# benattal/neural-radiance-caching

Measured on AMD Instinct MI355X. Metric: rays/sec (1024-ray batch, 64+64 proposal + 32 shaded samples/ray), hotdog cache forward, higher is better.
Workload: dtype f32

## Files before the change

### neural-radiance-caching_amd/csrc/rc_dev_mlp.h

```cpp
#pragma once
#include "rc_internal.h"

namespace rcdev {

typedef float f32x16 __attribute__((ext_vector_type(16)));

constexpr int kWaves = 4;

__device__ __forceinline__ f32x16 zero16() {
  f32x16 z;
#pragma unroll
  for (int i = 0; i < 16; ++i) z[i] = 0.0f;
  return z;
}

typedef uint32_t u32x4 __attribute__((ext_vector_type(4)));
typedef __bf16 bf16x8 __attribute__((ext_vector_type(8)));

__device__ __forceinline__ uint32_t pack_top16(float a1, float a0) {
  return __builtin_amdgcn_perm(__float_as_uint(a1), __float_as_uint(a0), 0x07060302u);
}
__device__ __forceinline__ float top16(float a) { return __uint_as_float(__float_as_uint(a) & 0xffff0000u); }
__device__ __forceinline__ void split8(const float (&v)[8], u32x4 (&b)[3]) {
  u32x4 &hi = b[0], &mid = b[1], &lo = b[2];
#pragma unroll
  for (int p = 0; p < 4; ++p) {
    const float a0 = v[2 * p], a1 = v[2 * p + 1];
    hi[p] = pack_top16(a1, a0);
    const float r0 = a0 - top16(a0), r1 = a1 - top16(a1);
    mid[p] = pack_top16(r1, r0);
    const float l0 = r0 - top16(r0), l1 = r1 - top16(r1);
    lo[p] = pack_top16(l1, l0);
  }
}
__device__ __forceinline__ f32x16 mfma_bf16(const u32x4& a, const u32x4& b, const f32x16& c) {
  return __builtin_amdgcn_mfma_f32_32x32x16_bf16(__builtin_bit_cast(bf16x8, a), __builtin_bit_cast(bf16x8, b), c, 0, 0, 0);
}
#ifndef RC_RULE1
#define RC_RULE1 1
#endif
#ifndef RC_RULE2
#define RC_RULE2 1
#endif
#ifndef RC_RULE3
#define RC_RULE3 1
#endif
typedef float f32x4 __attribute__((ext_vector_type(4)));
__device__ __forceinline__ void split_fence() { if constexpr (RC_RULE1 != 0) __builtin_amdgcn_sched_barrier(0); }
__device__ __forceinline__ void split_keep(const u32x4& x) { if constexpr (RC_RULE2 != 0) asm volatile("" ::"v"(x)); }
__device__ __forceinline__ void split_keep3(const u32x4 (&x)[3]) { if constexpr (RC_RULE2 != 0) asm volatile("" ::"v"(x[0]), "v"(x[1]), "v"(x[2])); }
template <class WS>
__device__ __forceinline__ void split_flush(const WS& w, const u32x4& any) {
  if constexpr (RC_RULE3 == 0) return;
  __builtin_amdgcn_sched_barrier(0);
  w.sink = __builtin_amdgcn_mfma_f32_16x16x32_bf16(__builtin_bit_cast(bf16x8, any), __builtin_bit_cast(bf16x8, any), w.sink, 0, 0, 0);
  w.sink = __builtin_amdgcn_mfma_f32_16x16x32_bf16(__builtin_bit_cast(bf16x8, any), __builtin_bit_cast(bf16x8, any), w.sink, 0, 0, 0);
  __builtin_amdgcn_sched_barrier(0);
  asm volatile("s_nop 1" : "+v"(w.sink));
  __builtin_amdgcn_sched_barrier(0);
}
__device__ __forceinline__ void split_exclusive_simd() {
  if constexpr (kRcSplit) asm volatile("" ::: "v255", "a255");
}
__device__ __forceinline__ void mfma_split6(const u32x4 (&a)[3], const u32x4 (&b)[3], f32x16& acc) {
  split_fence();
  acc = mfma_bf16(a[2], b[0], acc);
  acc = mfma_bf16(a[0], b[2], acc);
  acc = mfma_bf16(a[1], b[1], acc);
  acc = mfma_bf16(a[1], b[0], acc);
  acc = mfma_bf16(a[0], b[1], acc);
  acc = mfma_bf16(a[0], b[0], acc);
  split_fence();
}

__device__ __forceinline__ void mfma_split3(const u32x4 (&a)[3], const u32x4& b0, f32x16& acc) {
  split_fence();
  acc = mfma_bf16(a[2], b0, acc);
  acc = mfma_bf16(a[1], b0, acc);
  acc = mfma_bf16(a[0], b0, acc);
  split_fence();
}

constexpr int kChunk = 64;
constexpr int kRingFloats = 2 * kChunk * 64;

typedef __attribute__((address_space(3))) void* lds_void_ptr;

struct WStream {
  const float* g;
  float* ring;
  int lane, wave;
  mutable f32x4 sink = {0.0f, 0.0f, 0.0f, 0.0f};
  __device__ WStream() = default;
  __device__ WStream(const float* g_, float* ring_, int lane_, int wave_) : g(g_), ring(ring_), lane(lane_), wave(wave_) {}
};

template <int NF, int W = kWaves, int CH = kChunk>
__device__ __forceinline__ void ws_issue(const WStream& w, int c) {
  static_assert(CH % (4 * W) == 0, "whole 1-KiB pieces per wave");
#pragma unroll
  for (int k = 0; k < CH / 4 / W; ++k) {
    const int i = w.wave + W * k;
    const int frag0 = c * CH + 4 * i;
    if (frag0 < NF) {
      const float* src = w.g + (size_t)frag0 * 64 + w.lane * 4;
      float* dst = w.ring + ((c & 1) * CH + 4 * i) * 64;
      __builtin_amdgcn_global_load_lds((const void*)src, (lds_void_ptr)dst, 16, 0, 0);
    }
  }
}

template <int NF, int W = kWaves, int CH = kChunk>
__device__ __forceinline__ void ws_begin(const WStream& w) {
  ws_issue<NF, W, CH>(w, 0);
  asm volatile("s_waitcnt vmcnt(0)" ::: "memory");
  __syncthreads();
  if (CH < NF) ws_issue<NF, W, CH>(w, 1);
}

template <int NF, int W = kWaves, int CH = kChunk>
__device__ __forceinline__ void ws_advance(const WStream& w, int c) {
  asm volatile("s_waitcnt vmcnt(0)" ::: "memory");
  __syncthreads();
  if ((c + 1) * CH < NF) ws_issue<NF, W, CH>(w, c + 1);
}

template <int NF, int W = kWaves, int CH = kChunk>
__device__ __forceinline__ float ws_read(const WStream& w, int f) {
  if (f > 0 && f % CH == 0) ws_advance<NF, W, CH>(w, f / CH);
  return w.ring[(f % (2 * CH)) * 64 + w.lane];
}

__device__ __forceinline__ u32x4 lds_piece(const float* p) { return *reinterpret_cast<const u32x4*>(p); }
template <int NF, int W = kWaves, int CH = kChunk>
__device__ __forceinline__ u32x4 ws_read4(const WStream& w, int f) {
  static_assert(CH % 4 == 0, "pieces never straddle a chunk");
  if (f > 0 && f % CH == 0) ws_advance<NF, W, CH>(w, f / CH);
  return lds_piece(w.ring + (f % (2 * CH)) * 64 + w.lane * 4);
}

struct WDirect {
  const float* g;
  int lane;
  mutable f32x4 sink = {0.0f, 0.0f, 0.0f, 0.0f};
};
template <int NF, int W = kWaves, int CH = kChunk>
__device__ __forceinline__ float ws_read(const WDirect& w, int f) { return w.g[(size_t)f * 64 + w.lane]; }
template <int NF, int W = kWaves, int CH = kChunk>
__device__ __forceinline__ u32x4 ws_read4(const WDirect& w, int f) { return *reinterpret_cast<const u32x4*>(w.g + (size_t)f * 64 + w.lane * 4); }

template <int NT, int KS, int FBASE, int NF, int SG, int W, int CH, class WS>
__device__ __forceinline__ void mlp_layer_f32(const WS& w, const float* act, f32x16 (&acc)[NT]) {
  constexpr int NG = (KS + SG - 1) / SG;
  float a[3][SG][NT], b[3][SG];
  auto load = [&](int g, int buf) {
#pragma unroll
    for (int d = 0; d < SG; ++d) {
      const int s = g * SG + d;
      if (s < KS) {
        b[buf][d] = act[s * 64];
#pragma unroll
        for (int t = 0; t < NT; ++t) {
          const int f = FBASE + s * NT + t;
          a[buf][d][t] = ws_read<NF, W, CH>(w, f);
        }
      }
    }
  };
  auto comp = [&](int g, int buf) {
#pragma unroll
    for (int d = 0; d < SG; ++d) {
      if (g * SG + d < KS) {
#pragma unroll
        for (int t = 0; t < NT; ++t)
          acc[t] = __builtin_amdgcn_mfma_f32_32x32x2f32(a[buf][d][t], b[buf][d], acc[t], 0, 0, 0);
      }
    }
  };
  load(0, 0);
  if (NG > 1) load(1, 1);
#pragma unroll
  for (int g = 0; g < NG; ++g) {
    if (g + 2 < NG) load(g + 2, (g + 2) % 3);
    __builtin_amdgcn_sched_barrier(0);
    comp(g, g % 3);
    __builtin_amdgcn_sched_barrier(0);
  }
}


template <int NBP>
__device__ __forceinline__ void split_blocks(const float* act, u32x4 (&pre)[NBP][3]) {
  float v[NBP][8];
#pragma unroll
  for (int q = 0; q < NBP; ++q)
#pragma unroll
    for (int j = 0; j < 8; ++j) v[q][j] = act[(8 * q + j) * 64];
#pragma unroll
  for (int q = 0; q < NBP; ++q) split8(v[q], pre[q]);
}
template <int NT, int KS, int FBASE, int NF, int W, int CH, int NBP, bool BIAS1, class WS>
__device__ __forceinline__ void mlp_layer_split(const WS& w, const float* act, f32x16 (&acc)[NT], const u32x4 (*pre)[3]) {
  static_assert(FBASE % 4 == 0, "split layers start on a 1-KiB piece");
  constexpr int NB = (KS + 7) / 8, NC = NB * NT;
  static_assert(NBP <= NB, "no more ready blocks than blocks");
  static_assert(!BIAS1 || KS % 8 == 1, "a bias block holds the bias step alone");
  float bv[8];
  u32x4 a[3][3], b[2][3];
  u32x4 b1;
  b1[0] = (BIAS1 && w.lane < 32) ? 0x00003f80u : 0u; b1[1] = 0u; b1[2] = 0u; b1[3] = 0u;
  auto from_act = [](int q) { return q < NB && q >= NBP && !(BIAS1 && q == NB - 1); };
  auto load_b = [&](int q) {
#pragma unroll
    for (int j = 0; j < 8; ++j) bv[j] = (8 * q + j < KS) ? act[(8 * q + j) * 64] : 0.0f;
  };
  auto load_a = [&](int cell) {
#pragma unroll
    for (int p = 0; p < 3; ++p) a[cell % 3][p] = ws_read4<NF, W, CH>(w, FBASE + (cell * 3 + p) * 4);
  };
  auto keep_b = [&](int q) {
    if (BIAS1 && q == NB - 1) split_keep(b1);
    else if (q < NBP) split_keep3(pre[q]);
    else split_keep3(b[q & 1]);
  };
  if (from_act(0)) load_b(0);
  load_a(0);
  if (NC > 1) load_a(1);
  if (from_act(0)) split8(bv, b[0]);
  if (from_act(1)) load_b(1);
#pragma unroll
  for (int q = 0; q < NB; ++q) {
#pragma unroll
    for (int t = 0; t < NT; ++t) {
      const int cell = q * NT + t;
      if (BIAS1 && q == NB - 1) mfma_split3(a[cell % 3], b1, acc[t]);
      else if (q < NBP) mfma_split6(a[cell % 3], pre[q], acc[t]);
      else mfma_split6(a[cell % 3], b[q & 1], acc[t]);
      if (cell >= 1) split_keep3(a[(cell - 1) % 3]);
      if (cell + 2 < NC) load_a(cell + 2);
      if (t == 0) {
        if (q >= 1) keep_b(q - 1);
        if (from_act(q + 1)) split8(bv, b[(q + 1) & 1]);
        if (from_act(q + 2)) load_b(q + 2);
      }
    }
  }
  if (BIAS1) split_flush(w, b1);
  else if (NB - 1 < NBP) split_flush(w, pre[NB - 1][0]);
  else split_flush(w, b[(NB - 1) & 1][0]);
  split_keep3(a[(NC - 1) % 3]);
  keep_b(NB - 1);
}

template <int NT, int KS, int FBASE, int NF, int SG = (NT >= 8 ? 1 : (NT >= 4 ? 2 : (NT >= 2 ? 4 : 8))), int W = kWaves, int CH = kChunk, class WS = WStream>
__device__ __forceinline__ void mlp_layer(const WS& w, const float* act, f32x16 (&acc)[NT]) {
  if constexpr (kRcSplit) mlp_layer_split<NT, KS, FBASE, NF, W, CH, 0, false>(w, act, acc, nullptr);
  else mlp_layer_f32<NT, KS, FBASE, NF, SG, W, CH, WS>(w, act, acc);
}

template <int NT, int KS, int FBASE, int NF, int NBP, bool BIAS1, int W = kWaves, int CH = kChunk, class WS = WStream>
__device__ __forceinline__ void mlp_layer_x(const WS& w, const float* act, f32x16 (&acc)[NT], const u32x4 (*pre)[3] = nullptr) {
  mlp_layer_split<NT, KS, FBASE, NF, W, CH, NBP, BIAS1>(w, act, acc, pre);
}

template <int NT, int KS, int FBASE, int NF, int SG = (NT >= 8 ? 1 : (NT >= 4 ? 2 : (NT >= 2 ? 4 : 8))), int W = kWaves, int CH = kChunk, class WS = WStream>
__device__ __forceinline__ void mlp_layer_d(const WS& w, const float* act, f32x16 (&acc)[NT]) {
  mlp_layer_f32<NT, KS, FBASE, NF, SG, W, CH, WS>(w, act, acc);
}

template <int NT, int FBASE, int NF, int W = kWaves, int CH = kChunk, class WS = WStream>
__device__ __forceinline__ void mlp_bias_step(const WS& w, f32x16 (&acc)[NT]) {
  if constexpr (kRcSplit) {
    u32x4 b1;
    b1[0] = w.lane < 32 ? 0x00003f80u : 0u; b1[1] = 0u; b1[2] = 0u; b1[3] = 0u;
    u32x4 a[NT][3];
#pragma unroll
    for (int t = 0; t < NT; ++t)
#pragma unroll
      for (int p = 0; p < 3; ++p) a[t][p] = ws_read4<NF, W, CH>(w, FBASE + (t * 3 + p) * 4);
#pragma unroll
    for (int t = 0; t < NT; ++t) {
      split_fence();
      acc[t] = mfma_bf16(a[t][2], b1, acc[t]);
      acc[t] = mfma_bf16(a[t][1], b1, acc[t]);
      acc[t] = mfma_bf16(a[t][0], b1, acc[t]);
      split_fence();
    }
    split_flush(w, b1);
#pragma unroll
    for (int t = 0; t < NT; ++t) split_keep3(a[t]);
    split_keep(b1);
    return;
  }
  const float one = w.lane < 32 ? 1.0f : 0.0f;
  float a[NT];
#pragma unroll
  for (int t = 0; t < NT; ++t) a[t] = ws_read<NF, W, CH>(w, FBASE + t);
#pragma unroll
  for (int t = 0; t < NT; ++t) acc[t] = __builtin_amdgcn_mfma_f32_32x32x2f32(a[t], one, acc[t], 0, 0, 0);
}

template <int PT, int NT, int KS, int FBASE, int NF, int SG = (NT * PT >= 8 ? 1 : (NT * PT >= 4 ? 2 : 4)), int W = kWaves, class WS = WStream>
__device__ __forceinline__ void mlp_layer_pt(const WS& w, const float* act, int tile_stride, f32x16 (&acc)[PT][NT]) {
  constexpr int NG = (KS + SG - 1) / SG;
  float a[3][SG][NT], b[3][SG][PT];
  auto load = [&](int g, int buf) {
#pragma unroll
    for (int d = 0; d < SG; ++d) {
      const int s = g * SG + d;
      if (s < KS) {
#pragma unroll
        for (int p = 0; p < PT; ++p) b[buf][d][p] = act[p * tile_stride + s * 64];
#pragma unroll
        for (int t = 0; t < NT; ++t) {
          const int f = FBASE + s * NT + t;
          a[buf][d][t] = ws_read<NF, W, kChunk>(w, f);
        }
      }
    }
  };
  auto comp = [&](int g, int buf) {
#pragma unroll
    for (int d = 0; d < SG; ++d) {
      if (g * SG + d < KS) {
#pragma unroll
        for (int t = 0; t < NT; ++t)
#pragma unroll
          for (int p = 0; p < PT; ++p)
            acc[p][t] = __builtin_amdgcn_mfma_f32_32x32x2f32(a[buf][d][t], b[buf][d][p], acc[p][t], 0, 0, 0);
      }
    }
  };
  load(0, 0);
  if (NG > 1) load(1, 1);
#pragma unroll
  for (int g = 0; g < NG; ++g) {
    if (g + 2 < NG) load(g + 2, (g + 2) % 3);
    __builtin_amdgcn_sched_barrier(0);
    comp(g, g % 3);
    __builtin_amdgcn_sched_barrier(0);
  }
}

__device__ __forceinline__ float relu0(float x) {
  if constexpr (kRcSplit) {
    const int i = __float_as_int(x);
    return __int_as_float(i > 0 ? i : 0);
  }
  float y;
  asm("v_max_f32_e32 %0, 0, %1" : "=v"(y) : "v"(x));
  return y;
}

template <int NT, bool RELU>
__device__ __forceinline__ void park(const f32x16 (&acc)[NT], float* act, int base) {
#pragma unroll
  for (int t = 0; t < NT; ++t)
#pragma unroll
    for (int r = 0; r < 16; ++r) {
      const float v = acc[t][r];
      act[(base + t * 16 + r) * 64] = RELU ? relu0(v) : v;
    }
}

template <int PT, int NT, int NO, int FBASE, int NF, bool KEEP = false, int W = kWaves, int NOB = NO, int CH = kChunk, class WS = WStream>
__device__ __forceinline__ void dot_out(const WS& w, const f32x16 (&hid)[PT][NT], float (&out)[PT][NO],
                                        float (&keep)[KEEP ? NT * 16 : 1]) {
  float part[PT][NO][2];
#pragma unroll
  for (int p = 0; p < PT; ++p)
#pragma unroll
    for (int o = 0; o < NO; ++o) { part[p][o][0] = 0.0f; part[p][o][1] = 0.0f; }
#pragma unroll
  for (int o = 0; o < NO; ++o)
#pragma unroll
    for (int t = 0; t < NT; ++t)
#pragma unroll
      for (int r = 0; r < 16; ++r) {
        const float wv = ws_read<NF, W, CH>(w, FBASE + (o * NT + t) * 16 + r);
        if constexpr (KEEP) { if (o == 0) keep[t * 16 + r] = wv; }
#pragma unroll
        for (int p = 0; p < PT; ++p) part[p][o][r & 1] = __builtin_fmaf(relu0(hid[p][t][r]), wv, part[p][o][r & 1]);
      }
#pragma unroll
  for (int o = 0; o < NO; ++o) {
    const float bias = ws_read<NF, W, CH>(w, FBASE + NOB * NT * 16 + o);
#pragma unroll
    for (int p = 0; p < PT; ++p) {
      float sum = part[p][o][0] + part[p][o][1];
      sum = sum + __shfl_xor(sum, 32, 64);
      out[p][o] = sum + bias;
    }
  }
}
template <int NT, int NO, int FBASE, int NF, bool KEEP = false, int W = kWaves, int NOB = NO, int CH = kChunk, class WS = WStream>
__device__ __forceinline__ void dot_out1(const WS& w, const f32x16 (&hid)[NT], float (&out)[NO],
                                         float (&keep)[KEEP ? NT * 16 : 1]) {
  const f32x16 (&h1)[1][NT] = reinterpret_cast<const f32x16 (&)[1][NT]>(hid);
  float (&o1)[1][NO] = reinterpret_cast<float (&)[1][NO]>(out);
  dot_out<1, NT, NO, FBASE, NF, KEEP, W, NOB, CH, WS>(w, h1, o1, keep);
}

__device__ __forceinline__ float softplus(float x) {
  return fmaxf(x, 0.0f) + log1pf(expf(-fabsf(x)));
}
__device__ __forceinline__ float sigmoidf(float x) { return 1.0f / (1.0f + expf(-x)); }

#ifndef RC_DEV_CONTRACT3
#define RC_DEV_CONTRACT3
__device__ __forceinline__ void contract3(float& x, float& y, float& z, float radius) {
  x = rc_div(x, radius); y = rc_div(y, radius); z = rc_div(z, radius);
  float mag = x * x + y * y + z * z;
  mag = fmaxf(1.0f, mag);
  const float scale = (2.0f * sqrtf(mag) - 1.0f) / mag;
  x = scale * x; y = scale * y; z = scale * z;
}
#endif

__device__ __forceinline__ void neg_normalize(float& x, float& y, float& z) {
  const float dsq = x * x + y * y + z * z;
  const float inv = sqrtf(fmaxf(RC_TINY, dsq));
  float nx = -(x / inv), ny = -(y / inv), nz = -(z / inv);
  if (dsq < RC_TINY) { nx = 0.0f; ny = 0.0f; nz = 0.0f; }
  auto fix = [](float v) {
    if (v != v) return 0.0f;
    return fminf(fmaxf(v, -RC_FMAX), RC_FMAX);
  };
  x = fix(nx); y = fix(ny); z = fix(nz);
}


__host__ __device__ constexpr int ide_l(int i) { return i < 2 ? 1 : (i < 5 ? 2 : (i < 10 ? 4 : (i < 19 ? 8 : 16))); }
__host__ __device__ constexpr int ide_m(int i) { return i < 2 ? i : (i < 5 ? i - 2 : (i < 10 ? i - 5 : (i < 19 ? i - 10 : i - 19))); }


constexpr int kShActSteps = 102;
constexpr int kStepIde = 48;
constexpr int kStepBias = 84;

struct ShaderFrags {
  static constexpr int F_H = 0, F_S0 = F_H + rc_lfr(49, 1), F_I0 = F_S0 + rc_lfr(85, 8), F_I1 = F_I0 + rc_lfr(49, 2), F_IO = F_I1 + rc_lfr(33, 2),
                       F_S1 = F_IO + rc_dfr(1, 2), F_S2 = F_S1 + rc_lfr(65, 4), F_SB = F_S2 + rc_lfr(65, 4), F_SO = F_SB + rc_lfr(64, 4),
                       COUNT = F_SO + rc_dfr(3, 4);
};

struct ShaderConsts { float roughness_bias, irradiance_bias, ambient_bias, rgb_max, slf_ambient_bias; };
struct ShadeOut { float rgb[3], ad[3], idf[3], is[3], tint[3]; };

#ifdef RC_STAMPS
#define RC_TSTAMP(i) do { if (st) { __builtin_amdgcn_sched_barrier(0); st[i] = __builtin_amdgcn_s_memtime(); __builtin_amdgcn_sched_barrier(0); } } while (0)
#else
#define RC_TSTAMP(i) do { } while (0)
#endif
template <int F0, int NF, class WS = WStream>
__device__ __forceinline__ ShadeOut shader_tile(const WS& ws, float* act, int lane, int h, float nx, float ny, float nz,
                                                float vx, float vy, float vz, const RcIdeTable* tb, const ShaderConsts& k,
                                                unsigned long long* st = nullptr) {
  RC_TSTAMP(0);
  float rough, tint[3], ad[3], idf[3];
  u32x4 fpc[6][3];
  if constexpr (kRcSplit) split_blocks<6>(act, fpc);
  {
    f32x16 acc[1];
    acc[0] = zero16();
    if constexpr (kRcSplit) mlp_layer_x<1, 49, F0 + ShaderFrags::F_H, NF, 6, true>(ws, act, acc, fpc);
    else mlp_layer<1, 49, F0 + ShaderFrags::F_H, NF>(ws, act, acc);
    rough = softplus(acc[0][0] + k.roughness_bias);
    tint[0] = sigmoidf(acc[0][1]); tint[1] = sigmoidf(acc[0][2]); tint[2] = sigmoidf(acc[0][3]);
    const float ar[3] = {acc[0][4], acc[0][5], acc[0][6]};
    const float ir[3] = {acc[0][7], acc[0][8], acc[0][9]};
#pragma unroll
    for (int c = 0; c < 3; ++c) {
      ad[c] = fminf(fmaxf(softplus(ar[c] + k.ambient_bias), 0.0f), k.rgb_max);
      idf[c] = fminf(fmaxf(softplus(ir[c] + k.irradiance_bias), 0.0f), k.rgb_max);
    }
  }
  RC_TSTAMP(1);
  float dot_nv;
  {
    const float dotp = nx * (-vx) + ny * (-vy) + nz * (-vz);
    const float rx = 2.0f * dotp * nx - (-vx), ry = 2.0f * dotp * ny - (-vy), rz = 2.0f * dotp * nz - (-vz);
    act[kStepBias * 64] = h == 0 ? 1.0f : 0.0f;
    dot_nv = dotp;
    float zp[RC_IDE_ZPOW];
    zp[0] = 1.0f;
#pragma unroll
    for (int k = 1; k < RC_IDE_ZPOW; ++k) zp[k] = zp[k - 1] * rz;
    float cpw[RC_IDE_ZPOW];
    {
      float cre = 1.0f, cim = 0.0f;
      cpw[0] = h == 0 ? cre : cim;
#pragma unroll
      for (int m = 1; m < RC_IDE_ZPOW; ++m) {
        const float nre = cre * rx - cim * ry;
        const float nim = cre * ry + cim * rx;
        cre = nre; cim = nim;
        cpw[m] = h == 0 ? cre : cim;
      }
    }
#pragma unroll
    for (int i = 0; i < RC_IDE_TERMS; ++i) {
      const int l = ide_l(i), m = ide_m(i);
      float poly = 0.0f;
#pragma unroll
      for (int k = 0; k < RC_IDE_ZPOW; ++k) {
        if (k <= l - m && ((l - m - k) & 1) == 0) poly = poly + zp[k] * tb->coef[i][k];
      }
      const float att = expf(-(0.5f * (float)(l * (l + 1))) * rough);
      act[(kStepIde + i) * 64] = (cpw[m] * poly) * att;
    }
  }
  RC_TSTAMP(2);
  f32x16 s0[8];
#pragma unroll
  for (int t = 0; t < 8; ++t) s0[t] = zero16();
  if constexpr (kRcSplit) mlp_layer_x<8, 85, F0 + ShaderFrags::F_S0, NF, 6, false>(ws, act, s0, fpc);
  else mlp_layer<8, 85, F0 + ShaderFrags::F_S0, NF>(ws, act, s0);
  RC_TSTAMP(3);
  float ibrdf;
  {
    f32x16 ib[2];
    ib[0] = zero16(); ib[1] = zero16();
    act[48 * 64] = h == 0 ? dot_nv : 1.0f;
    if constexpr (kRcSplit) mlp_layer_x<2, 49, F0 + ShaderFrags::F_I0, NF, 6, false>(ws, act, ib, fpc);
    else mlp_layer<2, 49, F0 + ShaderFrags::F_I0, NF>(ws, act, ib);
    park<2, true>(ib, act, 48);
    act[(48 + 32) * 64] = h == 0 ? 1.0f : 0.0f;
    ib[0] = zero16(); ib[1] = zero16();
    if constexpr (kRcSplit) mlp_layer_x<2, 33, F0 + ShaderFrags::F_I1, NF, 0, true>(ws, act + 48 * 64, ib);
    else mlp_layer<2, 33, F0 + ShaderFrags::F_I1, NF>(ws, act + 48 * 64, ib);
    float o[1], nokeep[1];
    dot_out1<2, 1, F0 + ShaderFrags::F_IO, NF>(ws, ib, o, nokeep);
    ibrdf = sigmoidf(o[0] + 1.0986123f);
  }
  RC_TSTAMP(4);
  float amb[3];
  {
    f32x16 acc[4] = {s0[0], s0[1], s0[2], s0[3]};
    f32x16 skip[4] = {s0[4], s0[5], s0[6], s0[7]};
    park<4, true>(acc, act, 0);
    act[64 * 64] = h == 0 ? 1.0f : 0.0f;
#pragma unroll
    for (int t = 0; t < 4; ++t) acc[t] = zero16();
    if constexpr (kRcSplit) mlp_layer_x<4, 65, F0 + ShaderFrags::F_S1, NF, 0, true>(ws, act, acc);
    else mlp_layer<4, 65, F0 + ShaderFrags::F_S1, NF>(ws, act, acc);
    park<4, true>(acc, act, 0);
#pragma unroll
    for (int t = 0; t < 4; ++t) acc[t] = zero16();
    RC_TSTAMP(5);
    if constexpr (kRcSplit) mlp_layer_x<4, 65, F0 + ShaderFrags::F_S2, NF, 0, true>(ws, act, acc);
    else mlp_layer<4, 65, F0 + ShaderFrags::F_S2, NF>(ws, act, acc);
    park<4, true>(acc, act, 0);
    RC_TSTAMP(6);
    mlp_layer<4, 64, F0 + ShaderFrags::F_SB, NF>(ws, act, skip);
    RC_TSTAMP(7);
    float o[3], nokeep[1];
    dot_out1<4, 3, F0 + ShaderFrags::F_SO, NF>(ws, skip, o, nokeep);
#pragma unroll
    for (int c = 0; c < 3; ++c) amb[c] = fmaxf(softplus(o[c] + k.slf_ambient_bias), 0.0f);
  }
  RC_TSTAMP(8);
  ShadeOut o;
#pragma unroll
  for (int c = 0; c < 3; ++c) {
    const float is = fminf(fmaxf(tint[c] * ibrdf * (amb[c] * 1.0f), 0.0f), k.rgb_max);
    const float ambient = ad[c] + 0.0f;
    const float indirect = idf[c] + is;
    o.rgb[c] = ambient + indirect; o.ad[c] = ad[c]; o.idf[c] = idf[c]; o.is[c] = is; o.tint[c] = tint[c];
  }
  return o;
}

}
```

### neural-radiance-caching_amd/csrc/rc_fused.hip

```cpp
#include "rc_fused_common.h"
#include <type_traits>

using namespace rcdev;
using namespace rcfused;

namespace {

template <int K, int FB, int NF, class WS>
__device__ __forceinline__ float density_level64(const WS& ws, float* act_wave, int lane, const float (&f)[K]) {
  constexpr int KS0 = (K + 1) / 2 + 1;
  using FR = DensFrags<KS0>;
  const int tile = lane >> 5, j = lane & 31, h = lane >> 5;
#pragma unroll
  for (int k = 0; k < 2 * (KS0 - 1); ++k)
    act_wave[tile * kTileStride + (k >> 1) * 64 + j + 32 * (k & 1)] = k < K ? f[k < K ? k : 0] : 0.0f;
#pragma unroll
  for (int p = 0; p < 2; ++p) act_wave[p * kTileStride + (KS0 - 1) * 64 + lane] = h == 0 ? 1.0f : 0.0f;
  lds_sync<false>();
  float* act = act_wave + lane;
  f32x16 acc[2][2];
#pragma unroll
  for (int p = 0; p < 2; ++p) { acc[p][0] = zero16(); acc[p][1] = zero16(); }
  mlp_layer_pt<2, 2, KS0, FB + FR::D0, NF>(ws, act, kTileStride, acc);
#pragma unroll
  for (int p = 0; p < 2; ++p) { park<2, true>(acc[p], act + p * kTileStride, 0); act[p * kTileStride + 32 * 64] = h == 0 ? 1.0f : 0.0f; }
#pragma unroll
  for (int p = 0; p < 2; ++p) { acc[p][0] = zero16(); acc[p][1] = zero16(); }
  mlp_layer_pt<2, 2, 33, FB + FR::D1, NF>(ws, act, kTileStride, acc);
  float out[2][1], nokeep[1];
  dot_out<2, 2, 1, FB + FR::DO, NF>(ws, acc, out, nokeep);
  return tile == 0 ? out[0][0] : out[1][0];
}

template <bool GRAD, bool FRONT = false, bool DIRECT = false, bool EXPORT = false>
__global__ __launch_bounds__(kWaves * 64) void k_cache_fused(RcFusedArgs a) {
  split_exclusive_simd();
  constexpr int NF = FRONT ? F_SH : NF_FUSED;
  extern __shared__ __attribute__((aligned(16))) float lds_dyn[];
  const int wave = threadIdx.x >> 6, lane = threadIdx.x & 63;
  int64_t ray = (int64_t)blockIdx.x * kWaves + wave;
  const bool ray_ok = ray < a.n;
  if (!ray_ok) ray = a.n - 1;
  float* ring = lds_dyn;
  float* act_wave = lds_dyn + kRingFloats + wave * (kShActSteps * 64);
  float* scr = lds_dyn + kRingFloats + kWaves * (kShActSteps * 64) + wave * kScratch;
  float* s_sd[2] = {scr, scr + 68};
  float* s_td = scr + 2 * 68; float* s_cw = scr + 3 * 68; float* s_c = scr + 4 * 68; float* s_v = scr + 5 * 68;
  float* s_out = scr + 6 * 68;
  typename std::conditional<DIRECT, WDirect, WStream>::type ws;
  if constexpr (DIRECT) { ws.g = a.wstream; ws.lane = lane; }
  else { ws.g = a.wstream; ws.ring = ring; ws.lane = lane; ws.wave = wave; }
#ifdef RC_STAMPS
  unsigned long long stamps[16];
  const unsigned long long rt0 = __builtin_amdgcn_s_memrealtime();
#endif
  RC_FSTAMP(0);
  if constexpr (!DIRECT) ws_begin<NF>(ws);

  const float ox = a.origins[3 * ray], oy = a.origins[3 * ray + 1], oz = a.origins[3 * ray + 2];
  const float dx = a.directions[3 * ray], dy = a.directions[3 * ray + 1], dz = a.directions[3 * ray + 2];
  const float near = a.near[ray], far = a.far[ray];
  const float dnorm = sqrtf(dx * dx + dy * dy + dz * dz);

  auto resample = [&](int level, int P, int S, float logit, const float* s_prev) {
    const bool hasj = a.jitter[level] != nullptr;
    const float jit = hasj ? a.jitter[level][ray] : 0.0f;
#if defined(RC_ABL) && RC_ABL == 14
    for (int e2 = lane; e2 <= S; e2 += 64) s_out[e2] = (float)e2 / (float)S + 1e-9f * logit;
    lds_sync<false>();
#else
    sample_intervals_wave<false>(logit, P, S, a.us[level], hasj, jit, s_prev, s_cw, s_c, s_v, s_out, lane);
#endif
    if constexpr (FRONT) {
      if (a.use_raydist) {
        const float s_near = power_ladder(near, a.raydist_p, a.raydist_premult), s_far = power_ladder(far, a.raydist_p, a.raydist_premult);
        for (int e2 = lane; e2 <= S; e2 += 64)
          s_td[e2] = inv_power_ladder(s_out[e2] * s_far + (1.0f - s_out[e2]) * s_near, a.raydist_p, a.raydist_premult, a.y_max);
        lds_sync<false>();
        return;
      }
    }
    for (int e2 = lane; e2 <= S; e2 += 64) s_td[e2] = s_out[e2] * far + (1.0f - s_out[e2]) * near;
    lds_sync<false>();
  };
  auto mean_of = [&](int idx, float& mx, float& my, float& mz, float& t0, float& t1) {
    t0 = s_td[idx]; t1 = s_td[idx + 1];
    const float sm = t0 + t1, d = t1 - t0;
    const float ratio = (d * d) / fmaxf(RC_EPS * RC_EPS, 3.0f * (sm * sm) + d * d);
    const float tm = sm * (0.5f + ratio);
    mx = dx * tm + ox; my = dy * tm + oy; mz = dz * tm + oz;
  };
  auto density_of = [&](float raw, float cx, float cy, float cz, float bbox) {
    const bool inside = (cx > -bbox) & (cx < bbox) & (cy > -bbox) & (cy < bbox) & (cz > -bbox) & (cz < bbox);
    const float d = rc_safe_exp(raw + a.density_bias);
    return inside ? d : 0.0f;
  };

  if (lane == 0) { s_sd[0][0] = 0.0f; s_sd[0][1] = 1.0f; }
  lds_sync<false>();
  resample(0, 1, 64, a.anneal * safe_log(1.0f + a.padding), s_sd[0]);
  RC_FSTAMP(1);
  float w;
  {
    float mx, my, mz, t0, t1;
    mean_of(lane, mx, my, mz, t0, t1);
    float cx = mx, cy = my, cz = mz;
    contract3(cx, cy, cz, a.contract_radius);
    float f[6];
    {
      const float ux = unit_box(a.grid[0].bbox, cx), uy = unit_box(a.grid[0].bbox, cy), uz = unit_box(a.grid[0].bbox, cz);
#if defined(RC_ABL) && RC_ABL == 11
      for (int l = 0; l < 6; ++l) f[l] = ux * (float)l + uy - uz;
#else
      Corners<1> C[6];
      RC_FSTAMP(12);
#pragma unroll
      for (int l = 0; l < 6; ++l) {
        const RcGridLevel& L = a.grid[0].lvl[l];
        if (L.dense) grid_fetch_cell(a.cell_table[0][l], L.size, ux, uy, uz, C[l]);
        else grid_fetch<1, true>(L.table, L.size, L.mask, 0u, false, ux, uy, uz, C[l]);
      }
      RC_FSTAMP_NOWAIT(13);
      __builtin_amdgcn_sched_barrier(0);
#pragma unroll
      for (int l = 0; l < 6; ++l) {
        float v[1], jd[1];
        grid_combine<1, false>(C[l], v, jd);
        f[l] = v[0] * a.grid[0].precondition;
      }
#endif
    }
    RC_FSTAMP(2);
#if defined(RC_ABL) && RC_ABL == 13
    const float raw = f[0] + f[5];
#else
    const float raw = density_level64<6, F_L0, NF>(ws, act_wave, lane, f);
#endif
    w = alpha_weight(density_of(raw, cx, cy, cz, a.grid[0].bbox), t0, t1, dnorm, true, lane);
  }
  RC_FSTAMP(3);
  for (int e2 = lane; e2 <= 64; e2 += 64) s_sd[1][e2] = s_out[e2];
  lds_sync<false>();
  resample(1, 64, 64, a.anneal * safe_log(w + a.padding), s_sd[1]);
  RC_FSTAMP(4);
  {
    float mx, my, mz, t0, t1;
    mean_of(lane, mx, my, mz, t0, t1);
    float cx = mx, cy = my, cz = mz;
    contract3(cx, cy, cz, a.contract_radius);
    float f[7];
    {
      const float ux = unit_box(a.grid[1].bbox, cx), uy = unit_box(a.grid[1].bbox, cy), uz = unit_box(a.grid[1].bbox, cz);
#if defined(RC_ABL) && RC_ABL == 11
      for (int l = 0; l < 7; ++l) f[l] = ux * (float)l + uy - uz;
#else
      Corners<1> C[7];
#pragma unroll
      for (int l = 0; l < 7; ++l) {
        const RcGridLevel& L = a.grid[1].lvl[l];
        if (L.dense) grid_fetch_cell(a.cell_table[1][l], L.size, ux, uy, uz, C[l]);
        else grid_fetch<1, true>(L.table, L.size, L.mask, 0u, false, ux, uy, uz, C[l]);
      }
      __builtin_amdgcn_sched_barrier(0);
#pragma unroll
      for (int l = 0; l < 7; ++l) {
        float v[1], jd[1];
        grid_combine<1, false>(C[l], v, jd);
        f[l] = v[0] * a.grid[1].precondition;
      }
#endif
    }
    RC_FSTAMP(5);
#if defined(RC_ABL) && RC_ABL == 13
    const float raw = f[0] + f[6];
#else
    const float raw = density_level64<7, F_L1, NF>(ws, act_wave, lane, f);
#endif
    w = alpha_weight(density_of(raw, cx, cy, cz, a.grid[1].bbox), t0, t1, dnorm, true, lane);
  }
  RC_FSTAMP(6);
  for (int e2 = lane; e2 <= 64; e2 += 64) s_sd[0][e2] = s_out[e2];
  lds_sync<false>();
  resample(2, 64, 32, a.anneal * safe_log(w + a.padding), s_sd[0]);
  RC_FSTAMP(7);
  const int j = lane & 31, h = lane >> 5;
  float mx, my, mz, t0, t1;
  mean_of(j, mx, my, mz, t0, t1);
  float cx = mx, cy = my, cz = mz;
  const float zx = rc_div(mx, a.contract_radius), zy = rc_div(my, a.contract_radius), zz = rc_div(mz, a.contract_radius);
  contract3(cx, cy, cz, a.contract_radius);
  float* act = act_wave + lane;
  auto jac_at = [&](int e) -> float& { return act_wave[(kJac + (e >> 1)) * 64 + j + 32 * (e & 1)]; };
  {
    const RcGridDev& g = a.grid[2];
    float f[32];
    const float ux = unit_box(g.bbox, cx), uy = unit_box(g.bbox, cy), uz = unit_box(g.bbox, cz);
#if defined(RC_ABL) && RC_ABL == 11
    for (int k = 0; k < 32; ++k) f[k] = ux * (float)k + uy - uz;
    if (false)
#endif
#pragma unroll
    for (int half = 0; half < 2; ++half) {
      Corners<4> C[4];
#pragma unroll
      for (int q = 0; q < 4; ++q) {
        const int l = half * 4 + q;
        const RcGridLevel& L = a.grid[2].lvl[l];
        grid_fetch<4, true, 2, true>(a.pair_table[l] + 4 * h, L.size, L.mask, 0u, L.dense != 0, ux, uy, uz, C[q]);
      }
      __builtin_amdgcn_sched_barrier(0);
#pragma unroll
      for (int q = 0; q < 4; ++q) {
        const int l = half * 4 + q;
        const int size = a.grid[2].lvl[l].size;
        const bool dense = a.grid[2].lvl[l].dense != 0;
        float v[4], jd[GRAD ? 12 : 1];
        grid_combine<4, GRAD>(C[q], v, jd);
#pragma unroll
        for (int c = 0; c < 4; ++c) f[4 * l + c] = v[c] * g.precondition;
        if constexpr (GRAD) {
          const float s = g.precondition * (float)size / (2.0f * g.bbox);
          if (h == 0) {
#pragma unroll
            for (int c = 0; c < 4; ++c) {
              jac_at(0 * 32 + 4 * l + c) = (dense ? jd[2 * 4 + c] : jd[0 * 4 + c]) * s;
              jac_at(1 * 32 + 4 * l + c) = jd[1 * 4 + c] * s;
              jac_at(2 * 32 + 4 * l + c) = (dense ? jd[0 * 4 + c] : jd[2 * 4 + c]) * s;
            }
          }
        }
      }
    }
    const int base = h == 0 ? 0 : kAppTmp;
#pragma unroll
    for (int k = 0; k < 32; ++k) act_wave[(base + (k >> 1)) * 64 + j + 32 * (k & 1)] = f[k];
    act[16 * 64] = h == 0 ? 1.0f : 0.0f;
    lds_sync<false>();
  }
  RC_FSTAMP(8);
  using FR = DensFrags<17>;
  float density, npx, npy, npz, ngx = 0.0f, ngy = 0.0f, ngz = 0.0f;
  {
    f32x16 acc[2];
    acc[0] = zero16(); acc[1] = zero16();
    mlp_layer_d<2, 17, F_L2 + FR::D0, NF>(ws, act, acc);
    uint32_t m0 = 0, m1 = 0;
    if constexpr (GRAD) {
#pragma unroll
      for (int t = 0; t < 2; ++t)
#pragma unroll
        for (int r = 0; r < 16; ++r) m0 |= (acc[t][r] > 0.0f ? 1u : 0u) << (t * 16 + r);
    }
    park<2, true>(acc, act, 0);
    act[32 * 64] = h == 0 ? 1.0f : 0.0f;
    acc[0] = zero16(); acc[1] = zero16();
    mlp_layer_d<2, 33, F_L2 + FR::D1, NF>(ws, act, acc);
    if constexpr (GRAD) {
#pragma unroll
      for (int t = 0; t < 2; ++t)
#pragma unroll
        for (int r = 0; r < 16; ++r) m1 |= (acc[t][r] > 0.0f ? 1u : 0u) << (t * 16 + r);
    }
    park<2, true>(acc, act, 0);
    float out[4], wout[GRAD ? 32 : 1];
    dot_out1<2, 4, F_L2 + FR::DO, NF, GRAD>(ws, acc, out, wout);
    density = density_of(out[0], cx, cy, cz, a.grid[2].bbox);
    npx = out[1]; npy = out[2]; npz = out[3];
    neg_normalize(npx, npy, npz);
    if constexpr (GRAD) {
      float hid[32];
#pragma unroll
      for (int s = 0; s < 32; ++s) hid[s] = act[s * 64];
      float* bw = act;
#pragma unroll
      for (int s = 0; s < 32; ++s) bw[s * 64] = ((m1 >> s) & 1u) ? wout[s] : 0.0f;
      f32x16 g[2];
      g[0] = zero16(); g[1] = zero16();
      mlp_layer_d<2, 32, F_L2 + FR::B1, NF>(ws, bw, g);
#pragma unroll
      for (int t = 0; t < 2; ++t)
#pragma unroll
        for (int r = 0; r < 16; ++r) bw[(t * 16 + r) * 64] = ((m0 >> (t * 16 + r)) & 1u) ? g[t][r] : 0.0f;
      f32x16 gf[1];
      gf[0] = zero16();
      mlp_layer_d<1, 32, F_L2 + FR::B0, NF>(ws, bw, gf);
      float gp[3] = {0.0f, 0.0f, 0.0f};
#pragma unroll
      for (int r = 0; r < 16; ++r) {
        const int i = (r & 3) + 8 * (r >> 2) + 4 * h;
#pragma unroll
        for (int ax = 0; ax < 3; ++ax) gp[ax] += gf[0][r] * jac_at(ax * 32 + i);
      }
      float gw[3];
#pragma unroll
      for (int ax = 0; ax < 3; ++ax) {
        const float oth = __shfl_xor(gp[ax], 32, 64);
        gw[ax] = h == 0 ? gp[ax] + oth : oth + gp[ax];
      }
#pragma unroll
      for (int s = 0; s < 32; ++s) act[s * 64] = hid[s];
      const float msq = zx * zx + zy * zy + zz * zz;
      float gzx = gw[0], gzy = gw[1], gzz = gw[2];
      if (msq > 1.0f) {
        const float rt = sqrtf(msq);
        const float s = (2.0f * rt - 1.0f) / msq;
        const float ds = (1.0f - rt) / (msq * msq);
        const float gz_dot = gw[0] * zx + gw[1] * zy + gw[2] * zz;
        gzx = s * gw[0] + 2.0f * ds * gz_dot * zx;
        gzy = s * gw[1] + 2.0f * ds * gz_dot * zy;
        gzz = s * gw[2] + 2.0f * ds * gz_dot * zz;
      }
      ngx = rc_div(gzx, a.contract_radius); ngy = rc_div(gzy, a.contract_radius); ngz = rc_div(gzz, a.contract_radius);
      neg_normalize(ngx, ngy, ngz);
    } else if constexpr (!FRONT && !DIRECT) {
#pragma unroll
      for (int f = F_L2 + FR::B1; f < F_SH; ++f)
        if (f % kChunk == 0) ws_advance<NF>(ws, f / kChunk);
    }
  }
  RC_FSTAMP(9);
  if constexpr (FRONT) {
    if (ray_ok) {
      const int64_t np = a.n * 32, p = ray * 32 + j;
      for (int e2 = lane; e2 <= 32; e2 += 64) a.f_tdist[ray * 33 + e2] = s_td[e2];
      if (h == 0) {
        a.f_density[p] = density;
        a.f_means[p] = mx; a.f_means[np + p] = my; a.f_means[2 * np + p] = mz;
        a.f_normals_pred[p] = npx; a.f_normals_pred[np + p] = npy; a.f_normals_pred[2 * np + p] = npz;
        if constexpr (GRAD) {
          if (a.f_normals_grad) { a.f_normals_grad[p] = ngx; a.f_normals_grad[np + p] = ngy; a.f_normals_grad[2 * np + p] = ngz; }
        }
      }
      float* hb = a.f_hbuf + ray * (32 * 64) + lane;
#pragma unroll
      for (int s = 0; s < 32; ++s) hb[s * 64] = act[s * 64];
#pragma unroll
      for (int s = 0; s < 16; ++s) a.f_app[(int64_t)(2 * s + h) * np + p] = act[(kAppTmp + s) * 64];
    }
    return;
  }
  if constexpr (EXPORT) {
    if (ray_ok) {
      const int64_t np = a.n * 32, p = ray * 32 + j;
      for (int e2 = lane; e2 <= 32; e2 += 64) a.f_tdist[ray * 33 + e2] = s_td[e2];
      if (h == 0) {
        a.f_density[p] = density;
        a.f_means[p] = mx; a.f_means[np + p] = my; a.f_means[2 * np + p] = mz;
        a.f_normals_pred[p] = npx; a.f_normals_pred[np + p] = npy; a.f_normals_pred[2 * np + p] = npz;
      }
    }
  }
#pragma unroll
  for (int s = 0; s < 16; ++s) act[(32 + s) * 64] = act[(kAppTmp + s) * 64];
  act[48 * 64] = h == 0 ? 1.0f : 0.0f;
#if defined(RC_ABL) && RC_ABL == 12
  ShadeOut so;
  for (int c = 0; c < 3; ++c) { so.rgb[c] = act[c * 64]; so.ad[c] = npx; so.idf[c] = npy; so.is[c] = npz; so.tint[c] = density; }
#else
  const ShadeOut so = shader_tile<F_SH, NF>(ws, act, lane, h, npx, npy, npz, a.viewdirs[3 * ray], a.viewdirs[3 * ray + 1],
                                            a.viewdirs[3 * ray + 2], reinterpret_cast<const RcIdeTable*>(a.ide_coef), a.sh);
#endif

  RC_FSTAMP(10);
  const bool act_s = lane < 32;
  const float wnf = alpha_weight(density, t0, t1, dnorm, act_s, lane);
  auto store3 = [&](int id, float x, float y, float z) {
    if (lane == 0 && ray_ok && a.out.ptr[id]) { a.out.ptr[id][3 * ray] = x; a.out.ptr[id][3 * ray + 1] = y; a.out.ptr[id][3 * ray + 2] = z; }
  };
  auto store1 = [&](int id, float x) { if (lane == 0 && ray_ok && a.out.ptr[id]) a.out.ptr[id][ray] = x; };
  enum { V_ACC = 0, V_RGB = 1, V_AD = 4, V_IDF = 7, V_IS = 10, V_TINT = 13, V_DIF = 16, V_IND = 19, V_MEAN = 22, V_RD = 25,
         V_LD = 26, V_NP = 27, V_NG = 30, V_LOGT = 33, V_COUNT = 34 };
  float v[V_COUNT];
  v[V_ACC] = wnf;
#pragma unroll
  for (int c = 0; c < 3; ++c) {
    const float v_rgb = act_s ? so.rgb[c] : 0.0f, v_ad = act_s ? so.ad[c] : 0.0f, v_id = act_s ? so.idf[c] : 0.0f;
    const float v_is = act_s ? so.is[c] : 0.0f, v_t = act_s ? so.tint[c] : 0.0f;
    v[V_RGB + c] = wnf * v_rgb;
    v[V_AD + c] = wnf * v_ad;
    v[V_IDF + c] = wnf * v_id;
    v[V_IS + c] = wnf * v_is;
    v[V_TINT + c] = wnf * v_t;
    v[V_DIF + c] = wnf * (v_ad + v_id);
    v[V_IND + c] = wnf * (v_id + v_is);
  }
  v[V_MEAN] = wnf * mx; v[V_MEAN + 1] = wnf * my; v[V_MEAN + 2] = wnf * mz;
  v[V_RD] = wnf * sqrtf((ox - mx) * (ox - mx) + (oy - my) * (oy - my) + (oz - mz) * (oz - mz));
  v[V_LD] = 0.0f;
  if (a.lights) {
    const float lx = a.lights[3 * ray], ly = a.lights[3 * ray + 1], lz = a.lights[3 * ray + 2];
    v[V_LD] = wnf * sqrtf((lx - mx) * (lx - mx) + (ly - my) * (ly - my) + (lz - mz) * (lz - mz));
  }
  v[V_NP] = wnf * npx; v[V_NP + 1] = wnf * npy; v[V_NP + 2] = wnf * npz;
  v[V_NG] = wnf * ngx; v[V_NG + 1] = wnf * ngy; v[V_NG + 2] = wnf * ngz;
  v[V_LOGT] = act_s ? wnf * logf(0.5f * (t0 + t1)) : 0.0f;
  wave_sum_n<V_COUNT>(v);
  const float accw = v[V_ACC];
  const float bgw = fmaxf(0.0f, 1.0f - accw) * a.bg;
  store3(RC_OUT_RGB, v[V_RGB] + bgw, v[V_RGB + 1] + bgw, v[V_RGB + 2] + bgw);
  store3(RC_OUT_DIRECT_RGB, v[V_AD], v[V_AD + 1], v[V_AD + 2]);
  store3(RC_OUT_INDIRECT_DIFFUSE_RGB, v[V_IDF], v[V_IDF + 1], v[V_IDF + 2]);
  store3(RC_OUT_INDIRECT_SPECULAR_RGB, v[V_IS], v[V_IS + 1], v[V_IS + 2]);
  store3(RC_OUT_SPECULAR_RGB, v[V_IS], v[V_IS + 1], v[V_IS + 2]);
  store3(RC_OUT_ALBEDO_RGB, v[V_TINT], v[V_TINT + 1], v[V_TINT + 2]);
  store3(RC_OUT_DIFFUSE_RGB, v[V_DIF], v[V_DIF + 1], v[V_DIF + 2]);
  store3(RC_OUT_INDIRECT_RGB, v[V_IND], v[V_IND + 1], v[V_IND + 2]);
  store3(RC_OUT_INDIRECT_OCC, accw, accw, accw);
  store1(RC_OUT_ACC, accw);
  store3(RC_OUT_MEANS, v[V_MEAN], v[V_MEAN + 1], v[V_MEAN + 2]);
  store1(RC_OUT_RAY_DISTS, v[V_RD]);
  if (a.lights) store1(RC_OUT_LIGHT_DISTS, v[V_LD]);
  store3(RC_OUT_NORMALS_PRED, v[V_NP], v[V_NP + 1], v[V_NP + 2]);
  if constexpr (GRAD) store3(RC_OUT_NORMALS, v[V_NG], v[V_NG + 1], v[V_NG + 2]);
  {
    const float e = v[V_LOGT] / fmaxf(RC_EPS, accw);
    float dm = expf(e);
    if (dm != dm) dm = 0.0f;
    dm = fminf(dm, RC_FMAX);
    dm = fminf(fmaxf(dm, s_td[0]), s_td[32]);
    store1(RC_OUT_DISTANCE_MEAN, dm);
    const float wn = wnf / fmaxf(RC_EPS, accw);
    const float incl = wave_scan_incl(wn, lane);
    if (lane == 0) s_cw[0] = 0.0f;
    if (lane < 31) s_cw[lane + 1] = fminf(1.0f, incl);
    if (lane == 0) s_cw[32] = 1.0f;
    lds_sync<false>();
    if (lane < 3 && ray_ok) {
      const float ps = a.pct[lane] / 100.0f;
      const float v = interp1(ps, s_cw, s_td, 33);
      const int id = lane == 0 ? RC_OUT_DISTANCE_PERCENTILE_5 : (lane == 1 ? RC_OUT_DISTANCE_MEDIAN : RC_OUT_DISTANCE_PERCENTILE_95);
      if (a.out.ptr[id]) a.out.ptr[id][ray] = v;
    }
  }
  RC_FSTAMP(11);
#ifdef RC_STAMPS
  if (lane == 0 && a.stamps && ray_ok) {
    unsigned long long* d = a.stamps + ray * 16;
    for (int i = 0; i < 12; ++i) d[i] = stamps[i];
    d[14] = rt0; d[15] = __builtin_amdgcn_s_memrealtime();
    d[12] = stamps[12]; d[13] = stamps[13];
  }
#endif
}

}

#ifdef RC_STAMPS
static unsigned long long* g_fused_stamps = nullptr;
extern "C" void* rc_debug_fused_stamps() { return g_fused_stamps; }
#endif

__global__ void k_build_cells(const float* __restrict__ src, int N, int F, float* __restrict__ dst, int dst_stride, int dst_off) {
  const int M = N + 3;
// ... 92 lines not shown
```

Measured before the change: 9.562 million.

## Feed hidden-layer activations to the next MFMA layer from registers instead of LDS

Adds a register-held activation carrier (BHand) and templates the MLP layer kernels on a B-operand functor. Hidden activations between consecutive layers in the shader, density and gradient MLPs are kept in registers instead of being parked in per-wave LDS and read back. The bias step becomes a synthesized constant element. This is meant to remove LDS store/load round trips and the sync they need between layers, at the cost of more live VGPRs and a possible drop in occupancy or register spills.

```diff
diff --git a/neural-radiance-caching_amd/csrc/rc_dev_mlp.h b/neural-radiance-caching_amd/csrc/rc_dev_mlp.h
--- a/neural-radiance-caching_amd/csrc/rc_dev_mlp.h
+++ b/neural-radiance-caching_amd/csrc/rc_dev_mlp.h
@@ -149,8 +149,28 @@
 template <int NF, int W = kWaves, int CH = kChunk>
 __device__ __forceinline__ u32x4 ws_read4(const WDirect& w, int f) { return *reinterpret_cast<const u32x4*>(w.g + (size_t)f * 64 + w.lane * 4); }
 
-template <int NT, int KS, int FBASE, int NF, int SG, int W, int CH, class WS>
-__device__ __forceinline__ void mlp_layer_f32(const WS& w, const float* act, f32x16 (&acc)[NT]) {
+struct BAct {
+  const float* act;
+  __device__ __forceinline__ float operator()(int s) const { return act[s * 64]; }
+};
+template <int NT, bool BIAS>
+struct BHand {
+  float v[NT * 16];
+  float one;
+  __device__ __forceinline__ float operator()(int s) const { return s < NT * 16 ? v[s < NT * 16 ? s : 0] : one; }
+};
+struct BActPt {
+  const float* act; int tile_stride;
+  __device__ __forceinline__ float operator()(int p, int s) const { return act[p * tile_stride + s * 64]; }
+};
+template <int PT, int NT, bool BIAS>
+struct BHandPt {
+  BHand<NT, BIAS> hand[PT];
+  __device__ __forceinline__ float operator()(int p, int s) const { return hand[p](s); }
+};
+
+template <int NT, int KS, int FBASE, int NF, int SG, int W, int CH, class WS, class BF>
+__device__ __forceinline__ void mlp_layer_f32(const WS& w, const BF& bf, f32x16 (&acc)[NT]) {
   constexpr int NG = (KS + SG - 1) / SG;
   float a[3][SG][NT], b[3][SG];
   auto load = [&](int g, int buf) {
@@ -158,7 +178,7 @@
     for (int d = 0; d < SG; ++d) {
       const int s = g * SG + d;
       if (s < KS) {
-        b[buf][d] = act[s * 64];
+        b[buf][d] = bf(s);
 #pragma unroll
         for (int t = 0; t < NT; ++t) {
           const int f = FBASE + s * NT + t;
@@ -199,8 +219,8 @@
 #pragma unroll
   for (int q = 0; q < NBP; ++q) split8(v[q], pre[q]);
 }
-template <int NT, int KS, int FBASE, int NF, int W, int CH, int NBP, bool BIAS1, class WS>
-__device__ __forceinline__ void mlp_layer_split(const WS& w, const float* act, f32x16 (&acc)[NT], const u32x4 (*pre)[3]) {
+template <int NT, int KS, int FBASE, int NF, int W, int CH, int NBP, bool BIAS1, class WS, class BF>
+__device__ __forceinline__ void mlp_layer_split(const WS& w, const BF& bf, f32x16 (&acc)[NT], const u32x4 (*pre)[3]) {
   static_assert(FBASE % 4 == 0, "split layers start on a 1-KiB piece");
   constexpr int NB = (KS + 7) / 8, NC = NB * NT;
   static_assert(NBP <= NB, "no more ready blocks than blocks");
@@ -212,7 +232,7 @@
   auto from_act = [](int q) { return q < NB && q >= NBP && !(BIAS1 && q == NB - 1); };
   auto load_b = [&](int q) {
 #pragma unroll
-    for (int j = 0; j < 8; ++j) bv[j] = (8 * q + j < KS) ? act[(8 * q + j) * 64] : 0.0f;
+    for (int j = 0; j < 8; ++j) bv[j] = (8 * q + j < KS) ? bf(8 * q + j) : 0.0f;
   };
   auto load_a = [&](int cell) {
 #pragma unroll
@@ -254,18 +274,18 @@
 
 template <int NT, int KS, int FBASE, int NF, int SG = (NT >= 8 ? 1 : (NT >= 4 ? 2 : (NT >= 2 ? 4 : 8))), int W = kWaves, int CH = kChunk, class WS = WStream>
 __device__ __forceinline__ void mlp_layer(const WS& w, const float* act, f32x16 (&acc)[NT]) {
-  if constexpr (kRcSplit) mlp_layer_split<NT, KS, FBASE, NF, W, CH, 0, false>(w, act, acc, nullptr);
-  else mlp_layer_f32<NT, KS, FBASE, NF, SG, W, CH, WS>(w, act, acc);
+  if constexpr (kRcSplit) mlp_layer_split<NT, KS, FBASE, NF, W, CH, 0, false>(w, BAct{act}, acc, nullptr);
+  else mlp_layer_f32<NT, KS, FBASE, NF, SG, W, CH, WS>(w, BAct{act}, acc);
 }
 
 template <int NT, int KS, int FBASE, int NF, int NBP, bool BIAS1, int W = kWaves, int CH = kChunk, class WS = WStream>
 __device__ __forceinline__ void mlp_layer_x(const WS& w, const float* act, f32x16 (&acc)[NT], const u32x4 (*pre)[3] = nullptr) {
-  mlp_layer_split<NT, KS, FBASE, NF, W, CH, NBP, BIAS1>(w, act, acc, pre);
+  mlp_layer_split<NT, KS, FBASE, NF, W, CH, NBP, BIAS1>(w, BAct{act}, acc, pre);
 }
 
 template <int NT, int KS, int FBASE, int NF, int SG = (NT >= 8 ? 1 : (NT >= 4 ? 2 : (NT >= 2 ? 4 : 8))), int W = kWaves, int CH = kChunk, class WS = WStream>
 __device__ __forceinline__ void mlp_layer_d(const WS& w, const float* act, f32x16 (&acc)[NT]) {
-  mlp_layer_f32<NT, KS, FBASE, NF, SG, W, CH, WS>(w, act, acc);
+  mlp_layer_f32<NT, KS, FBASE, NF, SG, W, CH, WS>(w, BAct{act}, acc);
 }
 
 template <int NT, int FBASE, int NF, int W = kWaves, int CH = kChunk, class WS = WStream>
@@ -300,8 +320,8 @@
   for (int t = 0; t < NT; ++t) acc[t] = __builtin_amdgcn_mfma_f32_32x32x2f32(a[t], one, acc[t], 0, 0, 0);
 }
 
-template <int PT, int NT, int KS, int FBASE, int NF, int SG = (NT * PT >= 8 ? 1 : (NT * PT >= 4 ? 2 : 4)), int W = kWaves, class WS = WStream>
-__device__ __forceinline__ void mlp_layer_pt(const WS& w, const float* act, int tile_stride, f32x16 (&acc)[PT][NT]) {
+template <int PT, int NT, int KS, int FBASE, int NF, int SG, int W, class WS, class BF>
+__device__ __forceinline__ void mlp_layer_pt_b(const WS& w, const BF& bf, f32x16 (&acc)[PT][NT]) {
   constexpr int NG = (KS + SG - 1) / SG;
   float a[3][SG][NT], b[3][SG][PT];
   auto load = [&](int g, int buf) {
@@ -310,7 +330,7 @@
       const int s = g * SG + d;
       if (s < KS) {
 #pragma unroll
-        for (int p = 0; p < PT; ++p) b[buf][d][p] = act[p * tile_stride + s * 64];
+        for (int p = 0; p < PT; ++p) b[buf][d][p] = bf(p, s);
 #pragma unroll
         for (int t = 0; t < NT; ++t) {
           const int f = FBASE + s * NT + t;
@@ -342,6 +362,11 @@
   }
 }
 
+template <int PT, int NT, int KS, int FBASE, int NF, int SG = (NT * PT >= 8 ? 1 : (NT * PT >= 4 ? 2 : 4)), int W = kWaves, class WS = WStream>
+__device__ __forceinline__ void mlp_layer_pt(const WS& w, const float* act, int tile_stride, f32x16 (&acc)[PT][NT]) {
+  mlp_layer_pt_b<PT, NT, KS, FBASE, NF, SG, W, WS>(w, BActPt{act, tile_stride}, acc);
+}
+
 __device__ __forceinline__ float relu0(float x) {
   if constexpr (kRcSplit) {
     const int i = __float_as_int(x);
@@ -361,6 +386,30 @@
       const float v = acc[t][r];
       act[(base + t * 16 + r) * 64] = RELU ? relu0(v) : v;
     }
+}
+
+template <int NT, bool BIAS, bool RELU = true>
+__device__ __forceinline__ void hand_off(const f32x16 (&acc)[NT], int lane, BHand<NT, BIAS>& hb) {
+#pragma unroll
+  for (int t = 0; t < NT; ++t)
+#pragma unroll
+    for (int r = 0; r < 16; ++r) hb.v[t * 16 + r] = RELU ? relu0(acc[t][r]) : acc[t][r];
+  hb.one = lane < 32 ? 1.0f : 0.0f;
+}
+template <int NT, int NTP, bool BIAS, int FBASE, int NF, int W = kWaves, int CH = kChunk, class WS = WStream>
+__device__ __forceinline__ void mlp_layer_dh(const WS& w, const BHand<NTP, BIAS>& hb, f32x16 (&acc)[NT]) {
+  constexpr int SG = NT >= 8 ? 1 : (NT >= 4 ? 2 : (NT >= 2 ? 4 : 8));
+  mlp_layer_f32<NT, 16 * NTP + (BIAS ? 1 : 0), FBASE, NF, SG, W, CH, WS>(w, hb, acc);
+}
+template <int NT, int NTP, bool BIAS, int FBASE, int NF, int W = kWaves, int CH = kChunk, class WS = WStream>
+__device__ __forceinline__ void mlp_layer_h(const WS& w, const BHand<NTP, BIAS>& hb, f32x16 (&acc)[NT]) {
+  if constexpr (kRcSplit) mlp_layer_split<NT, 16 * NTP + (BIAS ? 1 : 0), FBASE, NF, W, CH, 0, BIAS>(w, hb, acc, nullptr);
+  else mlp_layer_dh<NT, NTP, BIAS, FBASE, NF, W, CH, WS>(w, hb, acc);
+}
+template <int PT, int NT, int NTP, bool BIAS, int FBASE, int NF, int W = kWaves, class WS = WStream>
+__device__ __forceinline__ void mlp_layer_pth(const WS& w, const BHandPt<PT, NTP, BIAS>& hb, f32x16 (&acc)[PT][NT]) {
+  constexpr int SG = NT * PT >= 8 ? 1 : (NT * PT >= 4 ? 2 : 4);
+  mlp_layer_pt_b<PT, NT, 16 * NTP + (BIAS ? 1 : 0), FBASE, NF, SG, W, WS>(w, hb, acc);
 }
 
 template <int PT, int NT, int NO, int FBASE, int NF, bool KEEP = false, int W = kWaves, int NOB = NO, int CH = kChunk, class WS = WStream>
@@ -524,11 +573,10 @@
     act[48 * 64] = h == 0 ? dot_nv : 1.0f;
     if constexpr (kRcSplit) mlp_layer_x<2, 49, F0 + ShaderFrags::F_I0, NF, 6, false>(ws, act, ib, fpc);
     else mlp_layer<2, 49, F0 + ShaderFrags::F_I0, NF>(ws, act, ib);
-    park<2, true>(ib, act, 48);
-    act[(48 + 32) * 64] = h == 0 ? 1.0f : 0.0f;
+    BHand<2, true> hi;
+    hand_off<2, true>(ib, lane, hi);
     ib[0] = zero16(); ib[1] = zero16();
-    if constexpr (kRcSplit) mlp_layer_x<2, 33, F0 + ShaderFrags::F_I1, NF, 0, true>(ws, act + 48 * 64, ib);
-    else mlp_layer<2, 33, F0 + ShaderFrags::F_I1, NF>(ws, act + 48 * 64, ib);
+    mlp_layer_h<2, 2, true, F0 + ShaderFrags::F_I1, NF>(ws, hi, ib);
     float o[1], nokeep[1];
     dot_out1<2, 1, F0 + ShaderFrags::F_IO, NF>(ws, ib, o, nokeep);
     ibrdf = sigmoidf(o[0] + 1.0986123f);
@@ -538,21 +586,20 @@
   {
     f32x16 acc[4] = {s0[0], s0[1], s0[2], s0[3]};
     f32x16 skip[4] = {s0[4], s0[5], s0[6], s0[7]};
-    park<4, true>(acc, act, 0);
-    act[64 * 64] = h == 0 ? 1.0f : 0.0f;
+    BHand<4, true> hs;
+    hand_off<4, true>(acc, lane, hs);
 #pragma unroll
     for (int t = 0; t < 4; ++t) acc[t] = zero16();
-    if constexpr (kRcSplit) mlp_layer_x<4, 65, F0 + ShaderFrags::F_S1, NF, 0, true>(ws, act, acc);
-    else mlp_layer<4, 65, F0 + ShaderFrags::F_S1, NF>(ws, act, acc);
-    park<4, true>(acc, act, 0);
+    mlp_layer_h<4, 4, true, F0 + ShaderFrags::F_S1, NF>(ws, hs, acc);
+    hand_off<4, true>(acc, lane, hs);
 #pragma unroll
     for (int t = 0; t < 4; ++t) acc[t] = zero16();
     RC_TSTAMP(5);
-    if constexpr (kRcSplit) mlp_layer_x<4, 65, F0 + ShaderFrags::F_S2, NF, 0, true>(ws, act, acc);
-    else mlp_layer<4, 65, F0 + ShaderFrags::F_S2, NF>(ws, act, acc);
-    park<4, true>(acc, act, 0);
+    mlp_layer_h<4, 4, true, F0 + ShaderFrags::F_S2, NF>(ws, hs, acc);
+    BHand<4, false> hb;
+    hand_off<4, false>(acc, lane, hb);
     RC_TSTAMP(6);
-    mlp_layer<4, 64, F0 + ShaderFrags::F_SB, NF>(ws, act, skip);
+    mlp_layer_h<4, 4, false, F0 + ShaderFrags::F_SB, NF>(ws, hb, skip);
     RC_TSTAMP(7);
     float o[3], nokeep[1];
     dot_out1<4, 3, F0 + ShaderFrags::F_SO, NF>(ws, skip, o, nokeep);
diff --git a/neural-radiance-caching_amd/csrc/rc_fused.hip b/neural-radiance-caching_amd/csrc/rc_fused.hip
--- a/neural-radiance-caching_amd/csrc/rc_fused.hip
+++ b/neural-radiance-caching_amd/csrc/rc_fused.hip
@@ -22,11 +22,12 @@
 #pragma unroll
   for (int p = 0; p < 2; ++p) { acc[p][0] = zero16(); acc[p][1] = zero16(); }
   mlp_layer_pt<2, 2, KS0, FB + FR::D0, NF>(ws, act, kTileStride, acc);
-#pragma unroll
-  for (int p = 0; p < 2; ++p) { park<2, true>(acc[p], act + p * kTileStride, 0); act[p * kTileStride + 32 * 64] = h == 0 ? 1.0f : 0.0f; }
+  BHandPt<2, 2, true> hd;
+#pragma unroll
+  for (int p = 0; p < 2; ++p) hand_off<2, true>(acc[p], lane, hd.hand[p]);
 #pragma unroll
   for (int p = 0; p < 2; ++p) { acc[p][0] = zero16(); acc[p][1] = zero16(); }
-  mlp_layer_pt<2, 2, 33, FB + FR::D1, NF>(ws, act, kTileStride, acc);
+  mlp_layer_pth<2, 2, 2, true, FB + FR::D1, NF>(ws, hd, acc);
   float out[2][1], nokeep[1];
   dot_out<2, 2, 1, FB + FR::DO, NF>(ws, acc, out, nokeep);
   return tile == 0 ? out[0][0] : out[1][0];
@@ -251,10 +252,12 @@
 #pragma unroll
         for (int r = 0; r < 16; ++r) m0 |= (acc[t][r] > 0.0f ? 1u : 0u) << (t * 16 + r);
     }
-    park<2, true>(acc, act, 0);
-    act[32 * 64] = h == 0 ? 1.0f : 0.0f;
-    acc[0] = zero16(); acc[1] = zero16();
-    mlp_layer_d<2, 33, F_L2 + FR::D1, NF>(ws, act, acc);
+    {
+      BHand<2, true> hd;
+      hand_off<2, true>(acc, lane, hd);
+      acc[0] = zero16(); acc[1] = zero16();
+      mlp_layer_dh<2, 2, true, F_L2 + FR::D1, NF>(ws, hd, acc);
+    }
     if constexpr (GRAD) {
 #pragma unroll
       for (int t = 0; t < 2; ++t)
@@ -268,22 +271,20 @@
     npx = out[1]; npy = out[2]; npz = out[3];
     neg_normalize(npx, npy, npz);
     if constexpr (GRAD) {
-      float hid[32];
-#pragma unroll
-      for (int s = 0; s < 32; ++s) hid[s] = act[s * 64];
-      float* bw = act;
-#pragma unroll
-      for (int s = 0; s < 32; ++s) bw[s * 64] = ((m1 >> s) & 1u) ? wout[s] : 0.0f;
+      BHand<2, false> bw;
+      bw.one = 0.0f;
+#pragma unroll
+      for (int s = 0; s < 32; ++s) bw.v[s] = ((m1 >> s) & 1u) ? wout[s] : 0.0f;
       f32x16 g[2];
       g[0] = zero16(); g[1] = zero16();
-      mlp_layer_d<2, 32, F_L2 + FR::B1, NF>(ws, bw, g);
+      mlp_layer_dh<2, 2, false, F_L2 + FR::B1, NF>(ws, bw, g);
 #pragma unroll
       for (int t = 0; t < 2; ++t)
 #pragma unroll
-        for (int r = 0; r < 16; ++r) bw[(t * 16 + r) * 64] = ((m0 >> (t * 16 + r)) & 1u) ? g[t][r] : 0.0f;
+        for (int r = 0; r < 16; ++r) bw.v[t * 16 + r] = ((m0 >> (t * 16 + r)) & 1u) ? g[t][r] : 0.0f;
       f32x16 gf[1];
       gf[0] = zero16();
-      mlp_layer_d<1, 32, F_L2 + FR::B0, NF>(ws, bw, gf);
+      mlp_layer_dh<1, 2, false, F_L2 + FR::B0, NF>(ws, bw, gf);
       float gp[3] = {0.0f, 0.0f, 0.0f};
 #pragma unroll
       for (int r = 0; r < 16; ++r) {
@@ -297,8 +298,6 @@
         const float oth = __shfl_xor(gp[ax], 32, 64);
         gw[ax] = h == 0 ? gp[ax] + oth : oth + gp[ax];
       }
-#pragma unroll
-      for (int s = 0; s < 32; ++s) act[s * 64] = hid[s];
       const float msq = zx * zx + zy * zy + zz * zz;
       float gzx = gw[0], gzy = gw[1], gzz = gw[2];
       if (msq > 1.0f) {
```

New measurement: 9.722 million, median of 6. 1.02x the previous value.
